# JSLeadbetter/julia-ocean-modelling

Measured on AMD Instinct MI355X. Metric: model timesteps/sec at N×N per GPU; achieved HBM GB/s vs roofline, 1/2/4/8 GPU, higher is better.
Workload: dtype f64

## Files before the change

include/qg_mi355.h:

```cpp
#ifndef QG_MI355_H
#define QG_MI355_H

#include <stdint.h>

#ifdef __cplusplus
extern "C" {
#endif

#define QG_ABI_VERSION 5

typedef enum {
    QG_OK = 0,
    QG_ERR_INVALID_ARG = -1,
    QG_ERR_UNSUPPORTED = -2,
    QG_ERR_HIP = -3,
    QG_ERR_NOT_BOUND = -4,
    QG_ERR_ALLOC = -5,
    QG_ERR_RCCL = -6,
    QG_ERR_NOT_CONVERGED = -7
} qg_status;

typedef enum {
    QG_SOLVER_SPECTRAL = 0,
    QG_SOLVER_PCG = 1
// ... 26 lines not shown
    double wind_rho0;
} qg_params;

typedef struct qg_ctx qg_ctx;
typedef struct qg_solver qg_solver;

typedef struct qg_stats {
    int32_t iters[2];
    double relres[2];
    double delta;
    double pin;
} qg_stats;

int qg_abi_version(void);
const char *qg_strerror(int status);
void qg_default_params(qg_params *p);

int qg_create(const qg_params *p, int device, void *stream, qg_ctx **out);
int qg_destroy(qg_ctx *ctx);
int qg_bind_state(qg_ctx *ctx, void *zeta, void *psi, void *f_store);
int qg_initialise(qg_ctx *ctx, uint64_t seed1, uint64_t seed2);
int qg_evolve_zeta(qg_ctx *ctx, int64_t timestep);
int qg_evolve_psi(qg_ctx *ctx);
int qg_step(qg_ctx *ctx, int64_t timestep);
int qg_run(qg_ctx *ctx, int64_t first_step, int64_t nsteps);
int qg_slot(const qg_ctx *ctx, int which, int logical, int *physical);
int qg_set_slots(qg_ctx *ctx, const int heads[3]);
int qg_canonicalize(qg_ctx *ctx);
#define QG_KEEP_ORDER_SLOT1 2
#define QG_KEEP_ORDER_SLOT1_DEFERRED 3
int qg_set_keep_order(qg_ctx *ctx, int on);
int qg_get_stats(qg_ctx *ctx, qg_stats *out);
int qg_set_pcg_sync(qg_ctx *ctx, int sync);
int qg_pcg_certificate(qg_ctx *ctx, int64_t *solves, int64_t *failures, int64_t *first_failure,
                       double *worst_relres);
int qg_solver_stats(qg_ctx *ctx, int *it_poisson, int *it_helm, double *relres_p, double *relres_h);
int qg_synchronize(qg_ctx *ctx);

int qg_snapshot(qg_ctx *ctx, void *host_zeta, void *host_psi);
int qg_snapshot_wait(qg_ctx *ctx);

typedef struct qg_diag {
    double zeta_max[2], zeta_min[2];
    double psi_max[2], psi_min[2];
    double zeta_sum[2];
    double enstrophy[2];
    double energy[2];
    double interface;
    double reserved;
} qg_diag;
int qg_diagnostics(qg_ctx *ctx, qg_diag *out);

int qg_comm_unique_id(char out[128]);
int qg_comm_init(qg_ctx *ctx, int nranks, int rank, const char id[128]);
typedef int (*qg_allgather_fn)(void *user, const double *send, double *recv, int64_t count, void *stream);
typedef int (*qg_sendrecv_fn)(void *user, int ns, const double *const *send, const int64_t *send_count,
                              const int *send_peer, int nr, double *const *recv, const int64_t *recv_count,
                              const int *recv_peer, void *stream);
int qg_comm_init_host(qg_ctx *ctx, int nranks, int rank, qg_allgather_fn allgather, qg_sendrecv_fn sendrecv,
                      void *user);
#define QG_PACE_STEPS 16
int qg_comm_set_timeout(qg_ctx *ctx, double seconds);
int qg_set_overlap(qg_ctx *ctx, int on);
enum { QG_HALO_RCCL = 0, QG_HALO_PEER = 1, QG_HALO_PUT = 2 };
int qg_comm_set_halo_transport(qg_ctx *ctx, int transport);
enum { QG_GATHER_RCCL = 0, QG_GATHER_PEER = 1 };
int qg_comm_set_gather_transport(qg_ctx *ctx, int transport);
int qg_comm_probe(qg_ctx *ctx, int reps, double out[4]);
enum { QG_XBUF_TO_NEXT = 0, QG_XBUF_TO_PREV = 1, QG_XBUF_FROM_PREV = 2, QG_XBUF_FROM_NEXT = 3 };
int qg_comm_exchange_plan(int rank, int nranks, int send_peer[2], int send_buf[2], int recv_peer[2],
                          int recv_buf[2]);

int qg_solver_create(int64_t M, int64_t P, double dx, const double alpha[2], const int pinned[2],
                     const double proj_in[4], const double proj_out[4], int kind, int precond,
                     int device, void *stream, qg_solver **out);
int qg_solver_solve(qg_solver *s, const double *f_1, const double *f_2, double *out_1, double *out_2);
int qg_solver_destroy(qg_solver *s);

enum {
    QG_FORM_TENDENCY = 0,
    QG_FORM_TENDENCY_TILE = 1,
    QG_FORM_ROW_SPLIT = 2,
    QG_FORM_PCG_NO_CERTIFICATE = 3,
    QG_FORM_COUNT = 4
};
enum { QG_TEND_AUTO = 0, QG_TEND_RING = 1, QG_TEND_DIRECT = 2, QG_TEND_ONE_POINT = 3 };
int qg_set_form(int which, int value);
int qg_get_form(int which);

int qg_laplace_5p(const double *u, double *out, int64_t M, int64_t P, double dx, void *stream);
int qg_cd(const double *u, double *out, int64_t M, int64_t P, double dx, void *stream);
int qg_arakawa_J(const double *zeta, const double *psi, double *out, int64_t M, int64_t P,
                 double dx, void *stream);
int qg_fill_ghosts(double *b, int64_t M, int64_t P, void *stream);

#ifdef __cplusplus
}
#endif
#endif
```

julia-ocean-modelling_amd/csrc/qg_capi.hip:

```cpp
#include <atomic>
#include <cmath>
#include <cstdlib>
#include <cstring>
#include <type_traits>
#include <vector>
#include <memory>
#include <new>

#include "qg_common.hpp"
#include "qg_mi355_profiles.h"
#include "qg_mi355_spectra.h"
#include "qg_mi355_spectra2d.h"
#include "qg_pcg.hpp"
#include "qg_spectral.hpp"
#include "qg_tracer.hpp"

namespace qg {
static std::atomic<int> g_form[QG_FORM_COUNT];
int form(int which) { return which >= 0 && which < QG_FORM_COUNT ? g_form[which].load(std::memory_order_relaxed) : 0; }
int comm_destroy(void *comm);
int comm_allgather(void *user, const double *send, double *recv, int64_t count, hipStream_t s);
int comm_halo(void *comm, double *const *fields, int nfields, int64_t M, int64_t P, int depth, double *halo_buf,
              hipStream_t s);
int comm_halo_rows(void *comm, double *const *f2, int n2, int64_t ld, int64_t P, hipStream_t s,
// ... 43 lines not shown
    size_t esize = 8;
    int heads[3] = {0, 0, 0};
    bool initialised = false;
    int seeded_rank = -1, seeded_nranks = -1;
    int rank = 0, nranks = 1;
    bool distributed = false;
    void *comm = nullptr;
    double *halo = nullptr;
    bool ghosts_pending = false;
    char *snap = nullptr;
    hipStream_t snap_stream = nullptr;
    hipEvent_t snap_ready = nullptr, snap_done = nullptr;
    bool snap_inflight = false;
    struct StepGraph {
        hipGraphExec_t exec = nullptr;
        int heads[3] = {0, 0, 0};
    };
    StepGraph graphs[3];
    int ngraphs = 0;
    bool graph_ok = true;
    hipStream_t gstream = nullptr;
    hipEvent_t gev_in = nullptr, gev_out = nullptr;
    bool overlap = true;
    hipStream_t ov_stream = nullptr;
    hipEvent_t ov_ready = nullptr, ov_halo = nullptr;
    hipEvent_t pace_ev = nullptr;
    bool pace_armed = false;
    int64_t pace_count = 0;
    int keep_order = 0;
    bool zcopy_pending = false;
    bool capturing = false;
    double *latch_host = nullptr;
    hipEvent_t latch_ev = nullptr;
    bool latch_armed = false;
    int64_t poll_count = 0;
    double *wind = nullptr;
    double *diag = nullptr;
    size_t diag_cap = 0;
    double *spectra = nullptr;
    double *spectra2d = nullptr;
    std::unique_ptr<SpectralSolver> spec;
    std::unique_ptr<PcgSolver> pcg;
    int last_status = QG_OK;
    int pcg_sync = -1;
    int64_t cert_reported = 0;
    size_t F = 0;

    void *fieldv(void *base, int layer, int slot) const {
        return static_cast<char *>(base) + esize * F * (size_t)(layer + 2 * slot);
    }
    double *field(void *base, int layer, int slot) const { return static_cast<double *>(fieldv(base, layer, slot)); }
    template <class T>
    T *fieldt(void *base, int layer, int slot) const { return static_cast<T *>(fieldv(base, layer, slot)); }
    int64_t row_words() const { return (int64_t)((p.M + 2) * esize / 8); }
};

void qg::tracer_owner(const qg_ctx *c, TracerOwner *o) {
    *o = TracerOwner{};
    o->M = c->p.M;
    o->P = c->p.P;
    o->dx = c->p.dx;
    o->dt = c->p.dt;
    o->U = c->p.U;
    o->device = c->device;
    o->stream = c->stream;
    o->F = c->F;
    o->bound = c->initialised && c->zeta;
    o->supported = c->esize == sizeof(double) && !c->distributed && c->nranks == 1 && c->p.M >= 3 && c->p.P >= 3;
    if (o->bound && o->supported)
        for (int l = 0; l < 2; ++l) {
            o->psi[l] = c->field(c->psi, l, c->heads[1]);
            o->zeta[l] = c->field(c->zeta, l, c->heads[0]);
        }
}

extern "C" {

int qg_abi_version(void) { return QG_ABI_VERSION; }

int qg_set_form(int which, int value) {
    if (which < 0 || which >= QG_FORM_COUNT || value < 0) return QG_ERR_INVALID_ARG;
    if (which == QG_FORM_TENDENCY && value > QG_TEND_ONE_POINT) return QG_ERR_INVALID_ARG;
    if ((which == QG_FORM_ROW_SPLIT || which == QG_FORM_PCG_NO_CERTIFICATE) && value > 1) return QG_ERR_INVALID_ARG;
    if (which == QG_FORM_TENDENCY_TILE && value != 0) {
        const int w = value >> 16, r = value & 0xffff;
        if ((w != 64 && w != 128 && w != 256 && w != 512) || r < 1) return QG_ERR_INVALID_ARG;
    }
    qg::g_form[which].store(value, std::memory_order_relaxed);
    return QG_OK;
}

int qg_get_form(int which) {
    if (which < 0 || which >= QG_FORM_COUNT) return QG_ERR_INVALID_ARG;
    return qg::form(which);
}

const char *qg_strerror(int s) {
    switch (s) {
        case QG_OK: return "ok";
        case QG_ERR_INVALID_ARG: return "invalid argument";
        case QG_ERR_UNSUPPORTED: return "unsupported configuration";
        case QG_ERR_HIP: return "HIP runtime error";
        case QG_ERR_NOT_BOUND: return "state not bound / not initialised";
        case QG_ERR_ALLOC: return "device allocation failed";
        case QG_ERR_RCCL: return "RCCL error or no communicator";
        case QG_ERR_NOT_CONVERGED: return "PCG did not converge";
        default: return "unknown status";
    }
}

void qg_default_params(qg_params *p) {
    if (!p) return;
    std::memset(p, 0, sizeof(*p));
    p->P_fwd[0] = 1.0;
    p->P_fwd[1] = -1.0;
    p->P_fwd[2] = 1.0;
    p->P_fwd[3] = 1.0;
    p->solver = QG_SOLVER_SPECTRAL;
    p->precond = QG_PRECOND_SPECTRAL;
    p->pcg_rtol = 1e-12;
    p->pcg_maxit = 500;
    p->chunk_rows = 0;
    p->wind_tau0 = 0.0;
    p->wind_rho0 = 1000.0;
}

static int check_params(const qg_params *p) {
    if (!p) return QG_ERR_INVALID_ARG;
    if (p->M < 2 || p->P < 2 || !(p->dx > 0) || !(p->H_1 > 0) || !(p->H_2 > 0) || !(p->R_d > 0))
        return QG_ERR_INVALID_ARG;
    if (p->solver != QG_SOLVER_SPECTRAL && p->solver != QG_SOLVER_PCG) return QG_ERR_INVALID_ARG;
    if (p->dtype != QG_F64 && p->dtype != QG_F32) return QG_ERR_INVALID_ARG;
    if (p->dtype == QG_F32 && (p->solver != QG_SOLVER_SPECTRAL || (p->M % 2) != 0)) return QG_ERR_UNSUPPORTED;
    if (p->wind_tau0 != 0 && !(p->wind_rho0 > 0)) return QG_ERR_INVALID_ARG;
    return QG_OK;
}

extern "C++" {
int qg::check_create_params(const qg_params *p) {
    QG_CHECK(check_params(p));
    const Derived d = derive(*p);
    if (!((d.beta1 > 0 && d.beta2 < 0) || (d.beta1 < 0 && d.beta2 > 0))) return QG_ERR_INVALID_ARG;
    return QG_OK;
}
}

static int ensure_wind(qg_ctx *c) {
    const qg_params &p = c->p;
    if (p.wind_tau0 == 0 || c->wind) return QG_OK;
    std::vector<double> w((size_t)p.P);
    const int64_t Pt = p.P * c->nranks, j0 = (int64_t)c->rank * p.P;
    for (int64_t j = 0; j < p.P; ++j) w[j] = wind_row(p.wind_tau0, p.wind_rho0, p.H_1, p.dx, Pt, j0 + j);
    QG_HIP(hipMalloc((void **)&c->wind, sizeof(double) * p.P));
    QG_HIP(hipMemcpy(c->wind, w.data(), sizeof(double) * p.P, hipMemcpyHostToDevice));
    return QG_OK;
}

static void drop_graphs(qg_ctx *c) {
    for (int g = 0; g < c->ngraphs; ++g)
        if (c->graphs[g].exec) (void)hipGraphExecDestroy(c->graphs[g].exec);
    c->ngraphs = 0;
}

static int build_solver(qg_ctx *c) {
    const qg_params &p = c->p;
    const double alpha[2] = {0.0, c->d.Seig};
// ... 1019 lines not shown
```

julia-ocean-modelling_amd/csrc/qg_stencil.hip:

```cpp
#include <algorithm>
#include <cstdio>
#include <cstdlib>

#include "qg_common.hpp"

namespace qg {

__global__ void laplace_kernel(const double *__restrict__ u, double *__restrict__ out, int64_t M,
                               int64_t P, double idx2) {
    const int64_t i = blockIdx.x * (int64_t)blockDim.x + threadIdx.x;
    const int64_t j = blockIdx.y;
    if (i >= M) return;
    const int64_t ld = M + 2, mi = i + 1, mj = j + 1;
    const double v = ((((u[fidx(mi - 1, mj, ld)] + u[fidx(mi + 1, mj, ld)]) - 4 * u[fidx(mi, mj, ld)]) +
                       u[fidx(mi, mj - 1, ld)]) + u[fidx(mi, mj + 1, ld)]) * idx2;
    store_with_ghosts(out, ld, M, P, i, j, v, true);
}

__global__ void cd_kernel(const double *__restrict__ u, double *__restrict__ out, int64_t M, int64_t P,
                          double c) {
    const int64_t i = blockIdx.x * (int64_t)blockDim.x + threadIdx.x;
    const int64_t j = blockIdx.y;
    if (i >= M) return;
    const int64_t ld = M + 2, mi = i + 1, mj = j + 1;
// ... 262 lines not shown
                if (layer == 1) {
#pragma unroll
                    for (int k = 0; k < 4; ++k) xch[j & 1][k][t] = part[k];
                } else {
#pragma unroll
                    for (int k = 0; k < 4; ++k) pend[k] = part[k];
                    pend_j = j;
                }
            }
        }
        {
            const LT p0 = rP[0], z0 = rZ[0], l0 = rL[0];
#pragma unroll
            for (int k = 0; k + 1 < RP; ++k) rP[k] = rP[k + 1];
#pragma unroll
            for (int k = 0; k + 1 < RZ; ++k) rZ[k] = rZ[k + 1];
#pragma unroll
            for (int k = 0; k + 1 < RL; ++k) rL[k] = rL[k + 1];
            rP[RP - 1] = p0;
            rZ[RZ - 1] = z0;
            rL[RL - 1] = l0;
        }
        nP += ld;
        nZ += ld;
        nF += ld;
        oRow += ld;
    }
    if constexpr (CERT) {
        __syncthreads();
        if (layer == 0) cert_fold();
        __shared__ double sv[4][2 * TX / 64];
        const int lane = threadIdx.x & 63, w = threadIdx.x >> 6;
#pragma unroll
        for (int k = 0; k < 4; ++k) {
            double v = cv[k];
#pragma unroll
            for (int o = 32; o > 0; o >>= 1) v += __shfl_xor(v, o, 64);
            if (lane == 0) sv[k][w] = v;
        }
        __syncthreads();
        if (threadIdx.x < 4) {
            double v = 0;
            for (int g = 0; g < 2 * TX / 64; ++g) v += sv[threadIdx.x][g];
            a.cert[4 * ((size_t)blockIdx.y * gridDim.x + blockIdx.x) + threadIdx.x] = v;
        }
    }
}

template <int TX, int PF, class T, bool CERT = false>
__global__ __launch_bounds__(CERT ? 2 * TX : TX, (CERT || TX >= 512) ? 4 : 5) void tendency_kernel(TendArgsT<T> a, int nyA, int nyB) {
    constexpr int RP = 6, RZ = 5, RL = 4;
    constexpr int NL = CERT ? 2 : 1;
    const TendBlock tb = tend_block();
    const int layer = CERT ? __builtin_amdgcn_readfirstlane((int)(threadIdx.x / TX)) : tb.z;
    const int t = CERT ? (int)(threadIdx.x % TX) : (int)threadIdx.x;
    const int M = (int)a.M;
    const int x0 = tb.x * TX;
    const int y = tb.y;
    const bool second = y >= nyA;
    const int r0 = second ? a.j2 : a.j0, nr = second ? a.j3 - a.j2 : a.j1 - a.j0;
    const int yy = second ? y - nyA : y, ny = second ? nyB : nyA;
    const int jb0 = r0 + (int)(((int64_t)yy * nr) / ny);
    const int jb1 = r0 + (int)(((int64_t)(yy + 1) * nr) / ny);
    if (jb0 >= jb1) {
        if constexpr (CERT) {
            if (threadIdx.x < 4) a.cert[4 * ((size_t)blockIdx.y * gridDim.x + blockIdx.x) + threadIdx.x] = 0;
        }
        return;
    }
    __shared__ T sp_[NL][RP][TX + 4];
    __shared__ T sz_[NL][RZ][TX + 2];
    __shared__ T sl_[NL][RL][TX + 2];
    __shared__ double xch[CERT ? 2 : 1][4][CERT ? TX : 1];
    const int L = CERT ? layer : 0;
    const bool in_rows = jb0 >= 2 && jb1 + 2 <= (int)a.P;
    if (x0 >= 2 && x0 + TX + 2 <= M) {
        if (in_rows) tendency_strip<TX, PF, T, CERT, false, true>(a, layer, t, x0, jb0, jb1, sp_[L], sz_[L], sl_[L], xch);
        else tendency_strip<TX, PF, T, CERT, false, false>(a, layer, t, x0, jb0, jb1, sp_[L], sz_[L], sl_[L], xch);
    } else {
        tendency_strip<TX, PF, T, CERT, true, false>(a, layer, t, x0, jb0, jb1, sp_[L], sz_[L], sl_[L], xch);
    }
}

template <class T>
struct PairT;
template <>
struct PairT<float> {
    typedef float V __attribute__((ext_vector_type(2)));
    typedef float VU __attribute__((ext_vector_type(2), aligned(4)));
};
template <>
struct PairT<double> {
    typedef double V __attribute__((ext_vector_type(2)));
    typedef double VU __attribute__((ext_vector_type(2), aligned(8)));
};

template <class T, bool EDGE = true>
__device__ __forceinline__ void store_pair_with_ghosts(T *row, T *grow, int M, int xa, T v0, T v1, bool has_b) {
    using VU = typename PairT<T>::VU;
    auto put = [&](T *r) {
        if constexpr (!EDGE) {
            *(VU *)(r + xa + 1) = VU{v0, v1};
            return;
        }
        if (has_b) {
            *(VU *)(r + xa + 1) = VU{v0, v1};
            if (xa + 1 == M - 1) r[0] = v1;
        } else {
            r[xa + 1] = v0;
            if (xa == M - 1) r[0] = v0;
        }
        if (xa == 0) r[M + 1] = v0;
    };
    put(row);
    if (grow) put(grow);
}

template <int TX, class T, int PF, bool EDGE, bool IN_ROWS>
__device__ __forceinline__ void tendency_pair_strip(const TendArgsT<T> &a, int layer, int x0, int jb0, int jb1,
                                                    T (*sp)[2 * TX + 4], T (*sz)[2 * TX + 4], T (*sl)[2 * TX + 4]) {
    using V = typename PairT<T>::V;
    using VU = typename PairT<T>::VU;
    constexpr int RP = 6, RZ = 5, RL = 4, W = 2 * TX;
    const int t = threadIdx.x;
    const int M = (int)a.M, P = (int)a.P;
    const int64_t ld = a.ld;
    const int xa = x0 + 2 * t;

    const T *psi = a.psi[layer];
    const T *zeta = a.zeta[layer];
    const RowSrcT<T> &prs = a.psi_rows[layer];
    const RowSrcT<T> &zrs = a.zeta_rows[layer];
    const T *const fp1 = a.fprev1[layer], *const fp2 = a.fprev2[layer];
    T *const zo = a.zeta_out[layer], *const fo = a.f_out[layer];
    T *const fs1 = a.fshift1[layer], *const fs2 = a.fshift2[layer];
    const double *const wind = layer == 0 ? a.wind : nullptr;
    const bool gr = a.write_ghost_rows != 0;
    const T dx = (T)a.dx, idx = T(1) / dx, idx2 = idx * idx;
    const T cdc = T(0.5) * idx;
    const T den = T(12) * (dx * dx);
    const T visc = (T)a.visc, dtT = (T)a.dt, Ut = (T)a.U, rt = (T)a.r;
    const bool small = M < W + 4;

    auto wx = [&](int x) -> int {
        if constexpr (!EDGE) return x;
        if (small) return ((x % M) + M) % M;
        return x < 0 ? x + M : (x >= M ? x - M : x);
    };
    auto rowp = [&](const T *base, const RowSrcT<T> &rs, int j) -> const T * {
        if (IN_ROWS || (j >= 0 && j < P)) return base + fidx(1, j + 1, ld);
        return rs.halo[j < 0 ? j + 2 : (j - P) + 2];
    };
    const int hq = t == 0 ? 0 : (t == TX - 1 ? W + 2 : -1);
    const int xh = t == 0 ? x0 - 2 : x0 + W;
    const bool has_a = !EDGE || xa < M, has_b = !EDGE || xa + 1 < M;
    const bool ab3 = a.ab3 != 0;
    const int c0 = 2 * t + 2;

    auto load_pair = [&](const T *r, V &c) {
        if (has_b) {
            const VU v = *(const VU *)(r + xa);
            c = V{v.x, v.y};
        } else {
            c = V{r[wx(xa)], r[wx(xa + 1)]};
        }
    };
// ... 454 lines not shown
    const int b = xcd_logical_id();
    const int x = b % nx;
    int r = b / nx;
    const int y = r % ny;
    r /= ny;
    const int layer = r & 1;
    const size_t off = (size_t)(r >> 1) * (size_t)mstride;
    const int i = x * 64 + (int)(threadIdx.x & 63);
    const int j = a.j0 + 4 * y + (int)(threadIdx.x >> 6);
    if (i >= (int)a.M || j >= a.j1) return;
    double zc, L0, P0;
    direct_point(a, layer, i, j, zc, L0, P0, off);
}

__global__ __launch_bounds__(256) void tendency_direct_sweep_kernel(TendArgsT<double> a, int nx, int ny, int64_t mstride,
                                                                    const TendMember *rec) {
    const int b = xcd_logical_id();
    const int x = b % nx;
    int r = b / nx;
    const int y = r % ny;
    r /= ny;
    const int layer = r & 1;
    const int m = r >> 1;
    const size_t off = (size_t)m * (size_t)mstride;
    const int i = x * 64 + (int)(threadIdx.x & 63);
    const int j = a.j0 + 4 * y + (int)(threadIdx.x >> 6);
    if (i >= (int)a.M || j >= a.j1) return;
    double zc, L0, P0;
    direct_point<double, true>(a, layer, i, j, zc, L0, P0, off, rec + m);
}

__global__ __launch_bounds__(256) void tendency_direct_cert_kernel(TendArgsT<double> a, int nyA, int nyB) {
    const TendBlock tb = tend_block();
    const int M = (int)a.M;
    const int i = tb.x * 64 + (int)(threadIdx.x & 63);
    const int w = (int)(threadIdx.x >> 6);
    const int y = tb.y;
    const bool second = y >= nyA;
    const int r0 = second ? a.j2 : a.j0, r1 = second ? a.j3 : a.j1;
    const int j = r0 + 4 * (second ? y - nyA : y) + w;
    double cv[4] = {0, 0, 0, 0};
    if (i < M && j < r1) {
        double part[2][4];
#pragma unroll
        for (int layer = 0; layer < 2; ++layer) {
            double zc, L0, P0;
            direct_point(a, layer, i, j, zc, L0, P0);
#pragma unroll
            for (int s = 0; s < 2; ++s) {
                const double b = -(a.cert_in[2 * s + layer] * zc);
                part[layer][2 * s] = b;
                part[layer][2 * s + 1] = b + a.cert_pinv[2 * s + layer] * (L0 + a.cert_alpha[s] * P0);
            }
        }
        double bs[2], rs[2];
#pragma unroll
        for (int s = 0; s < 2; ++s) {
            bs[s] = part[0][2 * s] + part[1][2 * s];
            rs[s] = part[0][2 * s + 1] + part[1][2 * s + 1];
        }
        if (a.cert_pin && i == 0 && j == 0) bs[0] = rs[0] = 0.0;
#pragma unroll
        for (int s = 0; s < 2; ++s) {
            cv[2 * s] = bs[s] * bs[s];
            cv[2 * s + 1] = rs[s] * rs[s];
        }
    }
    __shared__ double sv[4][4];
    const int lane = threadIdx.x & 63;
#pragma unroll
    for (int k = 0; k < 4; ++k) {
        double v = cv[k];
#pragma unroll
        for (int o = 32; o > 0; o >>= 1) v += __shfl_xor(v, o, 64);
        if (lane == 0) sv[k][w] = v;
    }
    __syncthreads();
    if (threadIdx.x < 4) {
        const double v = ((sv[threadIdx.x][0] + sv[threadIdx.x][1]) + sv[threadIdx.x][2]) + sv[threadIdx.x][3];
        a.cert[4 * ((size_t)blockIdx.y * gridDim.x + blockIdx.x) + threadIdx.x] = v;
    }
}

template <int TX, int PF, class T>
static int launch_tend_variant(const TendArgsT<T> &a, int rows, hipStream_t s) {
    const int nA = (a.j1 - a.j0 + rows - 1) / rows, nB = a.j3 > a.j2 ? (a.j3 - a.j2 + rows - 1) / rows : 0;
    dim3 grid((unsigned)((a.M + TX - 1) / TX), (unsigned)(nA + nB), 2);
    tendency_kernel<TX, PF, T><<<grid, TX, 0, s>>>(a, nA, nB);
    QG_LAUNCH_CHECK();
    return QG_OK;
}

template <class K>
static int tend_slots(K kernel, int threads, int &sl) {
    if (sl) return QG_OK;
    int dev = 0, cus = 0, per = 0;
    QG_HIP(hipGetDevice(&dev));
    QG_HIP(hipDeviceGetAttribute(&cus, hipDeviceAttributeMultiprocessorCount, dev));
    QG_HIP(hipOccupancyMaxActiveBlocksPerMultiprocessor(&per, kernel, threads, 0));
    sl = cus * (per > 0 ? per : 1);
    return QG_OK;
}

template <class T>
static int launch_tend_balanced(const TendArgsT<T> &a, hipStream_t s) {
    constexpr int TX = 256, PF = 1;
    static int sl = 0;
    QG_CHECK(tend_slots(tendency_kernel<TX, PF, T>, TX, sl));
    const int nx = (int)((a.M + TX - 1) / TX);
    const int rA = a.j1 - a.j0, rB = a.j3 > a.j2 ? a.j3 - a.j2 : 0;
    const double pts = (double)a.M * (rA + rB);
    const int waves = pts >= 40.0e6 ? 16 : (pts >= 12.0e6 ? 9 : (pts >= 3.0e6 ? 1 : 2));
    const int target = std::max(1, waves * sl / (2 * nx));
    auto split = [&](int rows) { return rows <= 0 ? 0 : std::max(1, std::min(rows / 4, (int)((int64_t)target * rows / (rA + rB)))); };
    const int nyA = split(rA), nyB = split(rB);
    dim3 grid((unsigned)nx, (unsigned)(nyA + nyB), 2);
    tendency_kernel<TX, PF, T><<<grid, TX, 0, s>>>(a, nyA, nyB);
    QG_LAUNCH_CHECK();
    return QG_OK;
}

template <int TX>
static int launch_tendency_cert_t(const TendArgsT<double> &a, int64_t cap, int *nblk, hipStream_t s) {
    constexpr int PF = 1;
    static int sl = 0;
    if (sl == 0) {
        int dev = 0, cus = 0, per = 0;
        QG_HIP(hipGetDevice(&dev));
        QG_HIP(hipDeviceGetAttribute(&cus, hipDeviceAttributeMultiprocessorCount, dev));
        QG_HIP(hipOccupancyMaxActiveBlocksPerMultiprocessor(&per, tendency_kernel<TX, PF, double, true>, 2 * TX, 0));
        sl = cus * (per > 0 ? per : 1);
    }
    const int nx = (int)((a.M + TX - 1) / TX);
    const int rA = a.j1 - a.j0, rB = a.j3 > a.j2 ? a.j3 - a.j2 : 0;
    const int waves = 3;
    const int target = std::max(1, waves * sl / nx);
    auto split = [&](int rows) { return rows <= 0 ? 0 : std::max(1, std::min(rows / 4, (int)((int64_t)target * rows / (rA + rB)))); };
    const int nyA = split(rA), nyB = split(rB);
    if (nyA + nyB == 0) {
        *nblk = 0;
        return QG_OK;
    }
    dim3 grid((unsigned)nx, (unsigned)(nyA + nyB), 1);
    if ((int64_t)grid.x * grid.y > cap) return QG_ERR_INVALID_ARG;
    tendency_kernel<TX, PF, double, true><<<grid, 2 * TX, 0, s>>>(a, nyA, nyB);
    QG_LAUNCH_CHECK();
    *nblk = (int)(grid.x * grid.y);
    return QG_OK;
}

constexpr double TEND_DIRECT_PTS = 1.2e6;

constexpr double CERT_DIRECT_PTS = 0.5e6;
int launch_tendency_cert(const TendArgsT<double> &a, int64_t cap, int *nblk, hipStream_t s) {
    const double pts = (double)a.M * ((a.j1 - a.j0) + (a.j3 > a.j2 ? a.j3 - a.j2 : 0));
    const int f = form(QG_FORM_TENDENCY);
    if (f == QG_TEND_DIRECT || (f != QG_TEND_RING && pts < CERT_DIRECT_PTS)) {
        const int nA = (a.j1 - a.j0 + 3) / 4, nB = a.j3 > a.j2 ? (a.j3 - a.j2 + 3) / 4 : 0;
        if (nA + nB == 0) {
            *nblk = 0;
            return QG_OK;
        }
        dim3 grid((unsigned)((a.M + 63) / 64), (unsigned)(nA + nB), 1);
        if ((int64_t)grid.x * grid.y > cap) return QG_ERR_INVALID_ARG;
        tendency_direct_cert_kernel<<<grid, 256, 0, s>>>(a, nA, nB);
        QG_LAUNCH_CHECK();
        *nblk = (int)(grid.x * grid.y);
        return QG_OK;
    }
    return launch_tendency_cert_t<128>(a, cap, nblk, s);
}

template <int TX, class T>
static int launch_tend_pair(const TendArgsT<T> &a, hipStream_t s) {
    constexpr int W = 2 * TX, PF = 1;
    static int sl = 0;
    QG_CHECK(tend_slots(tendency_pair_kernel<TX, T, PF>, TX, sl));
    const int nx = (int)((a.M + W - 1) / W);
    const double pts = (double)a.M * ((a.j1 - a.j0) + (a.j3 > a.j2 ? a.j3 - a.j2 : 0));
    const int waves = pts >= 40.0e6 ? 20 : 2;
    const int rA = a.j1 - a.j0, rB = a.j3 > a.j2 ? a.j3 - a.j2 : 0;
    const int target = std::max(1, waves * sl / (2 * nx));
    auto split = [&](int rows) { return rows <= 0 ? 0 : std::max(1, std::min(rows / 4, (int)((int64_t)target * rows / (rA + rB)))); };
    const int nyA = split(rA), nyB = split(rB);
    dim3 grid((unsigned)nx, (unsigned)(nyA + nyB), 2);
    tendency_pair_kernel<TX, T, PF><<<grid, TX, 0, s>>>(a, nyA, nyB);
    QG_LAUNCH_CHECK();
    return QG_OK;
}

static void tend_tile(int &w, int &r) {
    const int v = form(QG_FORM_TENDENCY_TILE);
    w = v >> 16;
    r = v & 0xffff;
    if ((w != 64 && w != 128 && w != 256 && w != 512) || r < 1) w = 0;
}

template <class T>
static int launch_tend_direct(const TendArgsT<T> &a, hipStream_t s) {
// ... 73 lines not shown
```

julia-ocean-modelling_amd/qgamd/_lib.py:

```python
from __future__ import annotations

import ctypes as C
import os

PKG_DIR = os.path.dirname(os.path.dirname(os.path.abspath(__file__)))
LIB_PATH = os.environ.get("QGMI355_LIB") or os.path.join(PKG_DIR, "lib", "libqgmi355.so")

QG_OK = 0
QG_ERR_INVALID_ARG, QG_ERR_UNSUPPORTED, QG_ERR_HIP, QG_ERR_NOT_BOUND = -1, -2, -3, -4
QG_ERR_ALLOC, QG_ERR_RCCL, QG_ERR_NOT_CONVERGED = -5, -6, -7
QG_ENS_MAX_MEMBERS = 65535
QG_SPEC_LINES, QG_SPEC_MAX_STRIPS = 5, 64
QG_PROF_LINES = 12
QG_TRACERS_MAX, QG_TRC_LINES = 8, 6
QG_TRC_FORM_AUTO, QG_TRC_FORM_RING, QG_TRC_FORM_ONE_POINT = 0, 1, 2
QG_FLT_LINES, QG_FLOATS_MAX_PER_LAYER = 8, 1 << 26
QG_FLT_PSI, QG_FLT_ZETA = 0, 1


def QG_TRC_FORM_RING_TILE(w, r):
    return (int(w) << 16) | (int(r) << 4) | QG_TRC_FORM_RING


QG_XBUF_TO_NEXT, QG_XBUF_TO_PREV, QG_XBUF_FROM_PREV, QG_XBUF_FROM_NEXT = 0, 1, 2, 3
QG_SOLVER_SPECTRAL = 0
QG_F64, QG_F32 = 0, 1
QG_SOLVER_PCG = 1
QG_PRECOND_NONE = 0
QG_PRECOND_SPECTRAL = 1
QG_PRECOND_MULTIGRID = 2
QG_KEEP_ORDER_SLOT1, QG_KEEP_ORDER_SLOT1_DEFERRED = 2, 3
QG_FORM_TENDENCY, QG_FORM_TENDENCY_TILE, QG_FORM_ROW_SPLIT, QG_FORM_PCG_NO_CERTIFICATE = 0, 1, 2, 3
QG_TEND_AUTO, QG_TEND_RING, QG_TEND_DIRECT, QG_TEND_ONE_POINT = 0, 1, 2, 3


class QgParams(C.Structure):

    _fields_ = [
        ("H_1", C.c_double), ("H_2", C.c_double), ("beta", C.c_double), ("Lx", C.c_double),
        ("Ly", C.c_double), ("dt", C.c_double), ("T", C.c_double), ("U", C.c_double),
        ("M", C.c_int64), ("P", C.c_int64),
        ("dx", C.c_double), ("visc", C.c_double), ("r", C.c_double), ("R_d", C.c_double),
        ("initial_kick", C.c_double),
        ("P_fwd", C.c_double * 4),
        ("solver", C.c_int32), ("precond", C.c_int32),
        ("pcg_rtol", C.c_double),
        ("pcg_maxit", C.c_int32), ("chunk_rows", C.c_int32),
        ("dtype", C.c_int32), ("reserved0", C.c_int32),
        ("wind_tau0", C.c_double), ("wind_rho0", C.c_double),
    ]


class QgDiag(C.Structure):
    _fields_ = [("zeta_max", C.c_double * 2), ("zeta_min", C.c_double * 2), ("psi_max", C.c_double * 2),
                ("psi_min", C.c_double * 2), ("zeta_sum", C.c_double * 2), ("enstrophy", C.c_double * 2),
                ("energy", C.c_double * 2), ("interface", C.c_double), ("reserved", C.c_double)]


class QgMemberParams(C.Structure):

    _fields_ = [("U", C.c_double), ("beta", C.c_double), ("r", C.c_double), ("visc", C.c_double),
                ("R_d", C.c_double), ("initial_kick", C.c_double), ("wind_tau0", C.c_double),
                ("reserved", C.c_double)]


class QgSpread(C.Structure):

    _fields_ = [("zeta_var", C.c_double * 2), ("psi_var", C.c_double * 2), ("zeta_mean_sq", C.c_double * 2),
                ("psi_mean_sq", C.c_double * 2), ("energy_spread", C.c_double * 2),
                ("energy_mean", C.c_double * 2), ("step", C.c_double), ("nmembers", C.c_double),
                ("reserved", C.c_double * 2)]


class QgTracerParams(C.Structure):

    _fields_ = [("layer", C.c_int32), ("reserved", C.c_int32), ("kappa", C.c_double), ("gamma", C.c_double)]


class QgStats(C.Structure):
    _fields_ = [("iters", C.c_int32 * 2), ("relres", C.c_double * 2), ("delta", C.c_double),
                ("pin", C.c_double)]


AllgatherFn = C.CFUNCTYPE(C.c_int, C.c_void_p, C.c_void_p, C.c_void_p, C.c_int64, C.c_void_p)
SendrecvFn = C.CFUNCTYPE(C.c_int, C.c_void_p, C.c_int, C.POINTER(C.c_void_p), C.POINTER(C.c_int64),
                         C.POINTER(C.c_int), C.c_int, C.POINTER(C.c_void_p), C.POINTER(C.c_int64),
                         C.POINTER(C.c_int), C.c_void_p)

_vp, _dp, _i64, _i32 = C.c_void_p, C.c_void_p, C.c_int64, C.c_int
SIGNATURES = [
    ("qg_abi_version", C.c_int, []),
    ("qg_strerror", C.c_char_p, [C.c_int]),
    ("qg_default_params", None, [C.POINTER(QgParams)]),
    ("qg_create", C.c_int, [C.POINTER(QgParams), C.c_int, _vp, C.POINTER(_vp)]),
    ("qg_destroy", C.c_int, [_vp]),
    ("qg_bind_state", C.c_int, [_vp, _dp, _dp, _dp]),
    ("qg_initialise", C.c_int, [_vp, C.c_uint64, C.c_uint64]),
    ("qg_evolve_zeta", C.c_int, [_vp, _i64]),
    ("qg_evolve_psi", C.c_int, [_vp]),
    ("qg_step", C.c_int, [_vp, _i64]),
    ("qg_run", C.c_int, [_vp, _i64, _i64]),
    ("qg_slot", C.c_int, [_vp, C.c_int, C.c_int, C.POINTER(C.c_int)]),
    ("qg_set_slots", C.c_int, [_vp, C.c_int * 3]),
    ("qg_canonicalize", C.c_int, [_vp]),
    ("qg_set_keep_order", C.c_int, [_vp, C.c_int]),
    ("qg_get_stats", C.c_int, [_vp, C.POINTER(QgStats)]),
    ("qg_solver_stats", C.c_int, [_vp, C.POINTER(C.c_int), C.POINTER(C.c_int), C.POINTER(C.c_double),
                                  C.POINTER(C.c_double)]),
    ("qg_synchronize", C.c_int, [_vp]),
    ("qg_snapshot", C.c_int, [_vp, _vp, _vp]),
    ("qg_snapshot_wait", C.c_int, [_vp]),
    ("qg_diagnostics", C.c_int, [_vp, C.POINTER(QgDiag)]),
    ("qg_comm_unique_id", C.c_int, [C.c_char_p]),
    ("qg_comm_init", C.c_int, [_vp, C.c_int, C.c_int, C.c_char_p]),
    ("qg_comm_init_host", C.c_int, [_vp, C.c_int, C.c_int, AllgatherFn, SendrecvFn, _vp]),
# ... 121 lines not shown
```

Baseline: 1844.

## Add sheared-strip f64 tendency kernel with diagonal column walk

Adds a new f64 tendency kernel in which each thread block walks its row strip along a diagonal, shifting its column origin by two per row so that tiles form a parallelogram. The origin is aligned to 16-element boundaries of the output, with a wraparound edge variant and a fallback to the existing strip kernel near the top and bottom boundaries. The aim is to spread halo reuse and balance load across adjacent blocks, and to improve alignment of streaming stores and loads. It is enabled automatically in the balanced launcher for large grids (at least 12M points) when M is divisible by 16 and by the tile width, and it can be forced on or off through a new form switch. The cost is wider LDS rows and more index arithmetic, which may reduce occupancy.

```diff
diff --git a/include/qg_mi355.h b/include/qg_mi355.h
--- a/include/qg_mi355.h
+++ b/include/qg_mi355.h
@@ -132,7 +132,8 @@
     QG_FORM_TENDENCY_TILE = 1,
     QG_FORM_ROW_SPLIT = 2,
     QG_FORM_PCG_NO_CERTIFICATE = 3,
-    QG_FORM_COUNT = 4
+    QG_FORM_TENDENCY_SHEAR = 4,
+    QG_FORM_COUNT = 5
 };
 enum { QG_TEND_AUTO = 0, QG_TEND_RING = 1, QG_TEND_DIRECT = 2, QG_TEND_ONE_POINT = 3 };
 int qg_set_form(int which, int value);
diff --git a/julia-ocean-modelling_amd/csrc/qg_capi.hip b/julia-ocean-modelling_amd/csrc/qg_capi.hip
--- a/julia-ocean-modelling_amd/csrc/qg_capi.hip
+++ b/julia-ocean-modelling_amd/csrc/qg_capi.hip
@@ -149,6 +149,7 @@
     if (which < 0 || which >= QG_FORM_COUNT || value < 0) return QG_ERR_INVALID_ARG;
     if (which == QG_FORM_TENDENCY && value > QG_TEND_ONE_POINT) return QG_ERR_INVALID_ARG;
     if ((which == QG_FORM_ROW_SPLIT || which == QG_FORM_PCG_NO_CERTIFICATE) && value > 1) return QG_ERR_INVALID_ARG;
+    if (which == QG_FORM_TENDENCY_SHEAR && value > 2) return QG_ERR_INVALID_ARG;
     if (which == QG_FORM_TENDENCY_TILE && value != 0) {
         const int w = value >> 16, r = value & 0xffff;
         if ((w != 64 && w != 128 && w != 256 && w != 512) || r < 1) return QG_ERR_INVALID_ARG;
diff --git a/julia-ocean-modelling_amd/csrc/qg_stencil.hip b/julia-ocean-modelling_amd/csrc/qg_stencil.hip
--- a/julia-ocean-modelling_amd/csrc/qg_stencil.hip
+++ b/julia-ocean-modelling_amd/csrc/qg_stencil.hip
@@ -368,6 +368,219 @@
     }
 }
 
+template <int TX, bool EDGE>
+__device__ __forceinline__ void tendency_strip_sheared(const TendArgsT<double> &a, int layer, int t, int o0, int jb0,
+                                                       int jb1, double (*sp)[TX + 8], double (*sz)[TX + 6],
+                                                       double (*sl)[TX + 4]) {
+    typedef double T;
+    constexpr int SH = 2, HP = 2 + SH, HZ = 1 + SH, HL = 1 + SH / 2;
+    constexpr int RP = 6, RZ = 5, RL = 4;
+    const int M = (int)a.M;
+    const int64_t ld = a.ld;
+    const T *const psi = a.psi[layer], *const zeta = a.zeta[layer];
+    const T *const fp1 = a.fprev1[layer], *const fp2 = a.fprev2[layer];
+    T *const zo = a.zeta_out[layer], *const fo = a.f_out[layer];
+    T *const fs1 = a.fshift1[layer], *const fs2 = a.fshift2[layer];
+    const double *const wind = layer == 0 ? a.wind : nullptr;
+    const T dx = (T)a.dx, idx = T(1) / dx, idx2 = idx * idx;
+    const T cdc = T(0.5) * idx;
+    const T den = T(12) * (dx * dx);
+    const T visc = (T)a.visc, dtT = (T)a.dt, Ut = (T)a.U, rt = (T)a.r;
+    const bool ab3 = a.ab3 != 0;
+
+    auto wx = [&](int x) -> int { return x < 0 ? x + M : (x >= M ? x - M : x); };
+    const int o0w = wx(o0);
+    auto org = [&](int j) -> int { return wx(o0w - SH * (j - jb0)); };
+    auto up = [&](int o) -> int { return o < SH ? o + M - SH : o - SH; };
+    auto rowoff = [&](int j) -> size_t {
+        return (size_t)(j + 1) * ld + 1 + (EDGE ? 0 : o0 - SH * (j - jb0));
+    };
+    const int64_t step = ld - (EDGE ? 0 : SH);
+
+    const int ph_q = t < HP ? t : (t >= TX - HP ? t + 2 * HP : -1);
+    const int zh_q = t < HZ ? t : (t >= TX - HZ ? t + 2 * HZ : -1);
+    auto col = [&](int o, int rel) -> int { return EDGE ? wx(o + rel) : rel; };
+    auto fetch_psi = [&](const T *r, int o, T &c, T &h) {
+        c = r[col(o, t)];
+        if (ph_q >= 0) h = r[col(o, ph_q - HP)];
+    };
+    auto fetch_zeta = [&](const T *r, int o, T &c, T &h) {
+        c = r[col(o, t)];
+        if (zh_q >= 0) h = r[col(o, zh_q - HZ)];
+    };
+    auto fetch_f = [&](size_t off, int o, T &g1, T &g2) {
+        if (ab3) {
+            g1 = ld_stream(fp1 + off + col(o, t));
+            g2 = ld_stream(fp2 + off + col(o, t));
+        }
+    };
+    auto commit_psi = [&](auto d, T c, T h) {
+        d[t + HP] = c;
+        if (ph_q >= 0) d[ph_q] = h;
+    };
+    auto commit_zeta = [&](auto d, T c, T h) {
+        d[t + HZ] = c;
+        if (zh_q >= 0) d[zh_q] = h;
+    };
+    auto lap_row = [&](auto pm, auto p0, auto pp, auto dst) {
+        for (int q = t; q < TX + 2 * HL; q += TX) {
+            const int c = q + (HP - HL);
+            dst[q] = ((((p0[c - 1] + p0[c + 1]) - T(4) * p0[c]) + pm[c - SH]) + pp[c + SH]) * idx2;
+        }
+    };
+    typedef __attribute__((address_space(3))) T *LT;
+    LT rP[RP], rZ[RZ], rL[RL];
+#pragma unroll
+    for (int k = 0; k < RP; ++k) rP[k] = (LT)sp[(jb0 - 2 + k + 2 * RP) % RP];
+#pragma unroll
+    for (int k = 0; k < RZ; ++k) rZ[k] = (LT)sz[(jb0 - 1 + k + 2 * RZ) % RZ];
+#pragma unroll
+    for (int k = 0; k < RL; ++k) rL[k] = (LT)sl[(jb0 - 1 + k + 2 * RL) % RL];
+
+    T pc = 0, ph = 0, zc = 0, zh = 0, f1 = 0, f2 = 0;
+    {
+        T p0c[5], p0h[5], z0c[3], z0h[3];
+#pragma unroll
+        for (int k = 0; k < 5; ++k) {
+            p0c[k] = p0h[k] = 0;
+            fetch_psi(psi + rowoff(jb0 - 2 + k), org(jb0 - 2 + k), p0c[k], p0h[k]);
+        }
+#pragma unroll
+        for (int k = 0; k < 3; ++k) {
+            z0c[k] = z0h[k] = 0;
+            fetch_zeta(zeta + rowoff(jb0 - 1 + k), org(jb0 - 1 + k), z0c[k], z0h[k]);
+        }
+#pragma unroll
+        for (int k = 0; k < 5; ++k) commit_psi(rP[k], p0c[k], p0h[k]);
+#pragma unroll
+        for (int k = 0; k < 3; ++k) commit_zeta(rZ[k], z0c[k], z0h[k]);
+    }
+    if (jb0 + 2 <= jb1) {
+        fetch_psi(psi + rowoff(jb0 + 3), org(jb0 + 3), pc, ph);
+        fetch_zeta(zeta + rowoff(jb0 + 2), org(jb0 + 2), zc, zh);
+    }
+    fetch_f(rowoff(jb0), o0w, f1, f2);
+    __syncthreads();
+    lap_row(rP[0], rP[1], rP[2], rL[0]);
+    lap_row(rP[1], rP[2], rP[3], rL[1]);
+    lap_row(rP[2], rP[3], rP[4], rL[2]);
+
+    const T *nP = psi + rowoff(jb0 + 4), *nZ = zeta + rowoff(jb0 + 3);
+    size_t nF = rowoff(jb0 + 1), oRow = rowoff(jb0);
+    int oP = org(jb0 + 4), oZ = org(jb0 + 3), oF = org(jb0 + 1), oO = o0w;
+
+    const T bl = (T)a.beta[layer];
+    for (int j = jb0; j < jb1; ++j) {
+        const bool more = j + 2 <= jb1;
+        if (more) {
+            commit_psi(rP[5], pc, ph);
+            commit_zeta(rZ[3], zc, zh);
+        }
+        const T f1c = f1, f2c = f2;
+        asm volatile("" : : "v"(f1c), "v"(f2c) : "memory");
+        if (j + 3 <= jb1) {
+            fetch_psi(nP, oP, pc, ph);
+            fetch_zeta(nZ, oZ, zc, zh);
+        }
+        if (j + 1 < jb1) fetch_f(nF, oF, f1, f2);
+        __syncthreads();
+        if (more) lap_row(rP[3], rP[4], rP[5], rL[3]);
+        {
+            const LT Lm = rL[0], L0 = rL[1], Lp = rL[2];
+            const LT Pm = rP[1], P0 = rP[2], Pp = rP[3];
+            const LT Zm = rZ[0], Z0 = rZ[1], Zp = rZ[2];
+            const int cl = t + HL, cz = t + HZ, cp = t + HP;
+            const T biharm = ((((L0[cl - 1] + L0[cl + 1]) - T(4) * L0[cl]) + Lm[cl - SH]) + Lp[cl + SH]) * idx2;
+            const T v_term = visc * biharm;
+            auto Z = [&](int da, int db) {
+                const LT r = db < 0 ? Zm : (db > 0 ? Zp : Z0);
+                return r[cz + da + SH * db];
+            };
+            auto S = [&](int da, int db) {
+                const LT r = db < 0 ? Pm : (db > 0 ? Pp : P0);
+                return r[cp + da + SH * db];
+            };
+            const T J_term = arakawa_point<T>(Z, S, den);
+            const T beta_term = bl * (cdc * (P0[cp + 1] - P0[cp - 1]));
+            T last;
+            if (layer == 0) last = Ut * (cdc * (Z0[cz + 1] - Z0[cz - 1]));
+            else last = rt * L0[cl];
+            T F = ((v_term - J_term) - beta_term) - last;
+            if (wind) F = F + (T)wind[j];
+            const T zcen = Z0[cz];
+            const T zn = ab3 ? zcen + dtT * ((((T)(23.0 / 12.0) * F) - ((T)(16.0 / 12.0) * f1c)) + ((T)(5.0 / 12.0) * f2c))
+                             : zcen + (dtT * F);
+            auto put = [&](T *out, T v) {
+                if constexpr (EDGE) store_row_with_ghosts<T, true>(out + oRow - 1, nullptr, M, col(oO, t), v);
+                else st_stream(out + oRow + t, v);
+            };
+            put(zo, zn);
+            put(fo, F);
+            if (ab3 && fs1) {
+                put(fs1, f1c);
+                put(fs2, f2c);
+            }
+        }
+        {
+            const LT p0 = rP[0], z0 = rZ[0], l0 = rL[0];
+#pragma unroll
+            for (int k = 0; k + 1 < RP; ++k) rP[k] = rP[k + 1];
+#pragma unroll
+            for (int k = 0; k + 1 < RZ; ++k) rZ[k] = rZ[k + 1];
+#pragma unroll
+            for (int k = 0; k + 1 < RL; ++k) rL[k] = rL[k + 1];
+            rP[RP - 1] = p0;
+            rZ[RZ - 1] = z0;
+            rL[RL - 1] = l0;
+        }
+        nP += step;
+        nZ += step;
+        nF += step;
+        oRow += step;
+        if constexpr (EDGE) {
+            oP = up(oP);
+            oZ = up(oZ);
+            oF = up(oF);
+            oO = up(oO);
+        }
+    }
+}
+
+template <int TX>
+__global__ __launch_bounds__(TX, TX >= 512 ? 4 : 5) void tendency_sheared_kernel(TendArgsT<double> a, int nyA, int nyB) {
+    constexpr int RP = 6, RZ = 5, RL = 4;
+    const TendBlock tb = tend_block();
+    const int layer = tb.z, t = (int)threadIdx.x;
+    const int M = (int)a.M, P = (int)a.P;
+    const int x0 = tb.x * TX;
+    const int y = tb.y;
+    const bool second = y >= nyA;
+    const int r0 = second ? a.j2 : a.j0, nr = second ? a.j3 - a.j2 : a.j1 - a.j0;
+    const int yy = second ? y - nyA : y, ny = second ? nyB : nyA;
+    const int jb0 = r0 + (int)(((int64_t)yy * nr) / ny);
+    const int jb1 = r0 + (int)(((int64_t)(yy + 1) * nr) / ny);
+    if (jb0 >= jb1) return;
+    __shared__ double lds[RP * (TX + 8) + RZ * (TX + 6) + RL * (TX + 4)];
+    if (jb0 >= 2 && jb1 + 2 <= P) {
+        double(*sp)[TX + 8] = (double(*)[TX + 8]) lds;
+        double(*sz)[TX + 6] = (double(*)[TX + 6])(lds + RP * (TX + 8));
+        double(*sl)[TX + 4] = (double(*)[TX + 4])(lds + RP * (TX + 8) + RZ * (TX + 6));
+        const uint64_t e = ((uint64_t)(uintptr_t)a.zeta_out[layer] >> 3) + (uint64_t)(jb0 + 1) * (uint64_t)a.ld + 1 + x0;
+        const int o0 = x0 + (int)((16 - (e & 15)) & 15);
+        const bool inside = o0 - 2 * (jb1 + 1 - jb0) - 4 >= 0 && o0 + 4 + TX + 4 <= M;
+        if (inside) tendency_strip_sheared<TX, false>(a, layer, t, o0, jb0, jb1, sp, sz, sl);
+        else tendency_strip_sheared<TX, true>(a, layer, t, o0, jb0, jb1, sp, sz, sl);
+    } else {
+        double(*sp)[TX + 4] = (double(*)[TX + 4]) lds;
+        double(*sz)[TX + 2] = (double(*)[TX + 2])(lds + RP * (TX + 4));
+        double(*sl)[TX + 2] = (double(*)[TX + 2])(lds + RP * (TX + 4) + RZ * (TX + 2));
+        double(*xch)[4][1] = nullptr;
+        const bool edge = x0 < 2 || x0 + TX + 2 > M;
+        if (edge) tendency_strip<TX, 1, double, false, true, false>(a, layer, t, x0, jb0, jb1, sp, sz, sl, xch);
+        else tendency_strip<TX, 1, double, false, false, false>(a, layer, t, x0, jb0, jb1, sp, sz, sl, xch);
+    }
+}
+
 template <class T>
 struct PairT;
 template <>
@@ -988,10 +1201,24 @@
     }
 }
 
+template <int TX>
+static bool tend_sheared(const TendArgsT<double> &a, bool automatic) {
+    const int f = form(QG_FORM_TENDENCY_SHEAR);
+    if (f == 1 || a.M % 16 != 0 || a.M % TX != 0 || a.M < 2 * TX) return false;
+    return f == 2 || automatic;
+}
+
 template <int TX, int PF, class T>
 static int launch_tend_variant(const TendArgsT<T> &a, int rows, hipStream_t s) {
     const int nA = (a.j1 - a.j0 + rows - 1) / rows, nB = a.j3 > a.j2 ? (a.j3 - a.j2 + rows - 1) / rows : 0;
     dim3 grid((unsigned)((a.M + TX - 1) / TX), (unsigned)(nA + nB), 2);
+    if constexpr (sizeof(T) == 8) {
+        if (tend_sheared<TX>(a, false)) {
+            tendency_sheared_kernel<TX><<<grid, TX, 0, s>>>(a, nA, nB);
+            QG_LAUNCH_CHECK();
+            return QG_OK;
+        }
+    }
     tendency_kernel<TX, PF, T><<<grid, TX, 0, s>>>(a, nA, nB);
     QG_LAUNCH_CHECK();
     return QG_OK;
@@ -1011,16 +1238,29 @@
 template <class T>
 static int launch_tend_balanced(const TendArgsT<T> &a, hipStream_t s) {
     constexpr int TX = 256, PF = 1;
-    static int sl = 0;
-    QG_CHECK(tend_slots(tendency_kernel<TX, PF, T>, TX, sl));
     const int nx = (int)((a.M + TX - 1) / TX);
     const int rA = a.j1 - a.j0, rB = a.j3 > a.j2 ? a.j3 - a.j2 : 0;
     const double pts = (double)a.M * (rA + rB);
+    bool sheared = false;
+    static int sl_straight = 0, sl_sheared = 0;
+    if constexpr (sizeof(T) == 8) {
+        sheared = tend_sheared<TX>(a, pts >= 12.0e6);
+        if (sheared) QG_CHECK(tend_slots(tendency_sheared_kernel<TX>, TX, sl_sheared));
+    }
+    if (!sheared) QG_CHECK(tend_slots(tendency_kernel<TX, PF, T>, TX, sl_straight));
+    const int sl = sheared ? sl_sheared : sl_straight;
     const int waves = pts >= 40.0e6 ? 16 : (pts >= 12.0e6 ? 9 : (pts >= 3.0e6 ? 1 : 2));
     const int target = std::max(1, waves * sl / (2 * nx));
     auto split = [&](int rows) { return rows <= 0 ? 0 : std::max(1, std::min(rows / 4, (int)((int64_t)target * rows / (rA + rB)))); };
     const int nyA = split(rA), nyB = split(rB);
     dim3 grid((unsigned)nx, (unsigned)(nyA + nyB), 2);
+    if constexpr (sizeof(T) == 8) {
+        if (sheared) {
+            tendency_sheared_kernel<TX><<<grid, TX, 0, s>>>(a, nyA, nyB);
+            QG_LAUNCH_CHECK();
+            return QG_OK;
+        }
+    }
     tendency_kernel<TX, PF, T><<<grid, TX, 0, s>>>(a, nyA, nyB);
     QG_LAUNCH_CHECK();
     return QG_OK;
diff --git a/julia-ocean-modelling_amd/qgamd/_lib.py b/julia-ocean-modelling_amd/qgamd/_lib.py
--- a/julia-ocean-modelling_amd/qgamd/_lib.py
+++ b/julia-ocean-modelling_amd/qgamd/_lib.py
@@ -31,6 +31,7 @@
 QG_PRECOND_MULTIGRID = 2
 QG_KEEP_ORDER_SLOT1, QG_KEEP_ORDER_SLOT1_DEFERRED = 2, 3
 QG_FORM_TENDENCY, QG_FORM_TENDENCY_TILE, QG_FORM_ROW_SPLIT, QG_FORM_PCG_NO_CERTIFICATE = 0, 1, 2, 3
+QG_FORM_TENDENCY_SHEAR = 4
 QG_TEND_AUTO, QG_TEND_RING, QG_TEND_DIRECT, QG_TEND_ONE_POINT = 0, 1, 2, 3
 
 
```

After: 1813. -1.7%, worse.
